# YonghaoHe/LFD-A-Light-and-Fast-Detector

Hardware: AMD Instinct MI355X
Metric: images/sec WIDERFACE-S 1920x1080 bs=8 end-to-end inference, LFD.precision='fp32_storage' (raw logits within 1e-4 of fp32: inside north_star's 1e-3; the 'fp16' mode, sigma 2.5e-3, under fp16_mode) (higher is better)
Workload: dtype f16

## Files before the change

### include/lfd_hip.h

```cpp
#ifndef LFD_HIP_H_
#define LFD_HIP_H_

#include <stddef.h>
#include <stdint.h>

#ifdef __cplusplus
extern "C" {
#endif

#define LFD_HIP_ABI_VERSION 3
#define LFD_MAX_LEVELS 8

typedef void* lfd_stream_t;

#if defined(LFD_BUILDING)
#define LFD_API __attribute__((visibility("default")))
#else
#define LFD_API
#endif

enum lfd_status {
  LFD_OK = 0,
  LFD_ERR_INVALID_ARGUMENT = -1,
  LFD_ERR_WORKSPACE_TOO_SMALL = -2,
// ... 315 lines not shown
  float gn_in_eps;
  int32_t pad_;
  int64_t f_image_stride0, f_image_stride1;
} lfd_pl_head_desc_t;
typedef struct lfd_pl_head_level {
  const void* in;
  void* out;
  const void* w0;
  const float* b0;
  const void* w1;
  const float* b1;
  void* gn_sums;
  const void* gn_in_sums;
  const float* gn_in_gamma;
  const float* gn_in_beta;
  float* f_out0;
  float* f_out1;
  const float* scale1;
  int64_t in_plane_halfs;
  int32_t pixels, pad_;
} lfd_pl_head_level_t;
LFD_API int lfd_pl_head_levels(const lfd_pl_head_desc_t* desc, const lfd_pl_head_level_t* levels, int32_t num_levels,
                               const void* zeros, lfd_stream_t stream);

LFD_API int lfd_stem_conv_f16(const void* in, int32_t in_format, int32_t n, int32_t h, int32_t w,
                              int32_t channels, const void* w1_packed, const float* b1,
                              const void* w2_packed, const float* b2, void* out, lfd_stream_t stream);

LFD_API int lfd_stem_gray_f16(const void* in, int32_t in_format, int32_t n, int32_t h, int32_t w, int32_t channels,
                              const void* w1_packed, const float* b1, const void* w2_packed, const float* b2, void* out,
                              lfd_stream_t stream);
LFD_API int lfd_pl_stem_gray_pair(const void* in, int32_t in_format, int32_t n, int32_t h, int32_t w, int32_t channels,
                                  const void* w1_packed, const float* b1, const void* w2_packed, const float* b2, void* out,
                                  int64_t out_plane_halfs, lfd_stream_t stream);

LFD_API int lfd_stem_faster_fused_f16(const void* in, int32_t in_format, int32_t n, int32_t h, int32_t w,
                                      int32_t channels, const void* w1_packed, const float* b1,
                                      const void* w2_packed, const float* b2, const void* w3_packed,
                                      const float* b3, const void* w4_packed, const float* b4, void* out,
                                      lfd_stream_t stream);

LFD_API size_t lfd_train_workspace_bytes(void);
LFD_API int lfd_pack_conv_weight_train_f16(const float* weight_oihw, int32_t cout, int32_t cin, int32_t ks, int32_t mode,
                                   int32_t rows_valid, void* packed, lfd_stream_t stream);
typedef struct lfd_pack_job {
  const float* w;
// ... 421 lines not shown
```

### lfd-a-light-and-fast-detector_amd/csrc/planes_head.hip

```cpp
#include "planes_impl.h"

namespace pl {

struct PhLevel {
  const void* in;
  long in_plane;
  float* out;
  const half8* w0;
  const float* b0;
  const half8* w1;
  const float* b1;
  unsigned long long* gn_out;
  const unsigned long long* gn_in;
  const float* gamma;
  const float* beta;
  float* f_out0;
  float* f_out1;
  const float* scale1;
  int P, tiles_per_img, tile_start, pad_;
};
struct PhArgs {
  PhLevel lv[LFD_MAX_LEVELS];
  const _Float16* zeros;
  long w_plane0, w_plane1;
  long f_img0, f_img1;
  int n_levels, N, ntiles, relu0;
  int f_c0, f_c1;
  float eps;
};

template <int MODE, int CIN, int NSLAB>
struct PhCfg {
  static constexpr int TPX = 64;
  static constexpr bool PLANES_IN = MODE == 0 || MODE == 3;
  static constexpr int NK0 = (PLANES_IN ? CIN : 128) / 16;
  static constexpr int IN_PIXB = CIN * 2;
  static constexpr int IN_PLANE = TPX * IN_PIXB;
  static constexpr int NBUF = ((MODE == 0 && CIN == 64) || MODE == 3) ? 2 : 1;
  static constexpr int RAW_BYTES = TPX * 512;
  static constexpr int OP_PLANE = TPX * 256;
  static constexpr int IN_OFF = 0;
  static constexpr int IN_BYTES = PLANES_IN ? NBUF * 2 * IN_PLANE : RAW_BYTES;
// ... 416 lines not shown
        const size_t pixi = in_img ? (size_t)px : 0;
        float* q0 = lv.f_out0 + (size_t)n * a.f_img0 + pixi * a.f_c0;
        float* q1 = lv.f_out1 + (size_t)n * a.f_img1 + pixi * a.f_c1 - a.f_c0;
#pragma unroll
        for (int g = 0; g < 4; ++g)
#pragma unroll
          for (int e = 0; e < 4; ++e) {
            if (slab * 32 + 8 * g + e < ctot) {
              const int co = slab * 32 + 8 * g + 4 * h + e;
              const float y = comb(am[0][4 * g + e], ac[0][4 * g + e]);
              const bool first_out = co < a.f_c0;
              float* dst = (in_img && co < ctot) ? (first_out ? q0 : q1) + co : trash;
              *dst = first_out ? y : y * sc1;
            }
          }
      }
    }
    if constexpr (PLANES_IN && C::NBUF == 2) buf ^= 1;
    PH_T(7);
  }
  gn_flush();
}

template <int NSLAB>
__global__ __launch_bounds__(256, 2) void k_pl_head_out(PhArgs a) {
  constexpr int TPX = 64, OP_PLANE = TPX * 256, BIAS_OFF = 4 * OP_PLANE;
  extern __shared__ __attribute__((aligned(16))) char smem[];
  const int lane = threadIdx.x & 63;
  const int wave = __builtin_amdgcn_readfirstlane((int)(threadIdx.x >> 6));
  const int h = lane >> 5, pix = lane & 31;
  const int slab = wave % NSLAB, pt0 = wave / NSLAB;
  const bool mfma_wave = wave < 2 * NSLAB;
  const int pj = (int)threadIdx.x & 31, gi = pj >> 1, prow = (int)threadIdx.x >> 5;
  const int nblk = gridDim.x;
  const int xcd = blockIdx.x & 7, bix = blockIdx.x >> 3;
  const int per_xcd = (a.ntiles + 7) / 8;
  const int x_begin = xcd * per_xcd;
  const int x_end = (x_begin + per_xcd) < a.ntiles ? (x_begin + per_xcd) : a.ntiles;
  const int wgs_xcd = (nblk + 7 - xcd) / 8;
  const int chunk = (x_end - x_begin + wgs_xcd - 1) / (wgs_xcd > 0 ? wgs_xcd : 1);
  const int t_first = x_begin + bix * chunk;
  const int t_last = (t_first + chunk) < x_end ? (t_first + chunk) : x_end;
  int lstart[LFD_MAX_LEVELS];
#pragma unroll
  for (int i = 0; i < LFD_MAX_LEVELS; ++i) lstart[i] = i < a.n_levels ? a.lv[i].tile_start : 0x7fffffff;
  auto level_of = [&](int t) {
    int l = 0;
#pragma unroll
// ... 10 lines not shown
  const char* d_in = nullptr;
  auto load_tile = [&](int t, float4* dst) {
    const int l = level_of(t);
    if (l != d_l) {
      d_l = l;
      with_level(l, [&](const PhLevel& v) { d_in = reinterpret_cast<const char*>(v.in); d_P = v.P; d_tpi = v.tiles_per_img; d_t0 = v.tile_start; });
    }
    const int rel = t - d_t0;
    const int n = rel / d_tpi;
    const int p0 = (rel - n * d_tpi) * TPX;
    const char* base = d_in + (long)n * d_P * 512 + pj * 16;
#pragma unroll
    for (int r = 0; r < 8; ++r) {
      int p = p0 + prow + 8 * r;
      p = p < d_P ? p : d_P - 1;
      dst[r] = *reinterpret_cast<const float4*>(base + (long)p * 512);
    }
  };
  float* sbias = reinterpret_cast<float*>(smem + BIAS_OFF);
  half8 wh[8], wl[8];
  float gn_a[4], gn_b[4];
  PhLevel lv{};
  int cur_l = -1, gnin_key = -1;
  const int xo = (pt0 * 32 + pix) * 256;
  const int xkey = (pix & 15) ^ h;
  float4 cur[8], nxt[8];
  int buf = 0;
  int t = t_first;
  if (t < t_last) load_tile(t, cur);
  for (; t < t_last; ++t, buf ^= 1) {
    const int l = level_of(t);
    if (l != cur_l) {
      cur_l = l;
      with_level(l, [&](const PhLevel& v) { lv = v; });
      const half8* ws = lv.w0 + ((size_t)slab * 8) * 64 + lane;
#pragma unroll
      for (int k = 0; k < 8; ++k) {
        wh[k] = ws[(size_t)k * 64];
        wl[k] = ws[a.w_plane0 + (size_t)k * 64];
      }
      block_barrier();
      if (threadIdx.x < 128) sbias[threadIdx.x] = ((int)threadIdx.x >= NSLAB * 32) ? 0.f : lv.b0[threadIdx.x];
      gnin_key = -1;
    }
    const int rel = t - lv.tile_start;
    const int n = rel / lv.tiles_per_img;
    const int p0 = (rel - n * lv.tiles_per_img) * TPX;
    if (t + 1 < t_last) load_tile(t + 1, nxt);
    if (gnin_key != n) {
      gnin_key = n;
      long long s = 0, q = 0;
#pragma unroll
      for (int r = 0; r < kGnRep; ++r) {
        s += (long long)lv.gn_in[(((size_t)r * a.N + n) * 16 + gi) * 2];
        q += (long long)lv.gn_in[(((size_t)r * a.N + n) * 16 + gi) * 2 + 1];
      }
      const double cnt = (double)lv.P * 8.0;
// ... 33 lines not shown
          ac[4 * g + 0] = 0.f; ac[4 * g + 1] = 0.f; ac[4 * g + 2] = 0.f; ac[4 * g + 3] = 0.f;
        }
      }
      const char* op = smem + buf * 2 * OP_PLANE + xo;
      half8 xh[2], xl[2];
      xh[0] = *reinterpret_cast<const half8*>(op + ((0 ^ xkey) << 4));
      xl[0] = *reinterpret_cast<const half8*>(op + OP_PLANE + ((0 ^ xkey) << 4));
      static_for([&](auto kc) {
        constexpr int k = decltype(kc)::value;
        if constexpr (k + 1 < 8) {
          xh[(k + 1) & 1] = *reinterpret_cast<const half8*>(op + (((2 * (k + 1)) ^ xkey) << 4));
          xl[(k + 1) & 1] = *reinterpret_cast<const half8*>(op + OP_PLANE + (((2 * (k + 1)) ^ xkey) << 4));
        }
        PL_SB();
        am = __builtin_amdgcn_mfma_f32_32x32x16_f16(wh[k], xh[k & 1], am, 0, 0, 0);
        ac = __builtin_amdgcn_mfma_f32_32x32x16_f16(wh[k], xl[k & 1], ac, 0, 0, 0);
        ac = __builtin_amdgcn_mfma_f32_32x32x16_f16(wl[k], xh[k & 1], ac, 0, 0, 0);
        PL_SB();
      }, std::make_integer_sequence<int, 8>{});
      const float sc1 = lv.scale1 ? *lv.scale1 : 1.f;
      const int ctot = a.f_c0 + a.f_c1;
      const int px = p0 + pt0 * 32 + pix;
      const bool in_img = px < lv.P;
      float* q0 = lv.f_out0 + (size_t)n * a.f_img0 + (size_t)px * a.f_c0;
      float* q1 = lv.f_out1 + (size_t)n * a.f_img1 + (size_t)px * a.f_c1 - a.f_c0;
#pragma unroll
      for (int g = 0; g < 4; ++g)
#pragma unroll
        for (int e = 0; e < 4; ++e) {
          if (slab * 32 + 8 * g + e < ctot) {
            const int co = slab * 32 + 8 * g + 4 * h + e;
            const float y = comb(am[4 * g + e], ac[4 * g + e]);
            if (in_img && co < ctot) {
              if (co < a.f_c0) q0[co] = y;
              else q1[co] = y * sc1;
            }
          }
        }
    }
#pragma unroll
    for (int r = 0; r < 8; ++r) cur[r] = nxt[r];
  }
}

template <int NSLAB>
int launch_pl_head_out(PhArgs& a, hipStream_t st) {
  long nt = 0;
  for (int i = 0; i < a.n_levels; ++i) {
    a.lv[i].tiles_per_img = (a.lv[i].P + 63) / 64;
    a.lv[i].tile_start = (int)nt;
    nt += (long)a.N * a.lv[i].tiles_per_img;
    if (nt > 0x7fffffffL) return LFD_ERR_UNSUPPORTED;
  }
  a.ntiles = (int)nt;
  constexpr int LDSB = 4 * 64 * 256 + 512;
  auto kern = k_pl_head_out<NSLAB>;
  static unsigned long long attr_done_mask = 0;
  const int attr_done_dev = lfd_device_ordinal();
  if (LFD_ONCE_PER_DEVICE(attr_done_mask, attr_done_dev)) {
    if (hipFuncSetAttribute(reinterpret_cast<const void*>(kern), hipFuncAttributeMaxDynamicSharedMemorySize, LDSB) != hipSuccess)
      return LFD_ERR_LAUNCH_FAILED;
    LFD_DONE_ON_DEVICE(attr_done_mask, attr_done_dev);
  }
  int blocks = 512;
  if (blocks > 8 * ((a.ntiles + 7) / 8)) blocks = 8 * ((a.ntiles + 7) / 8);
  if (blocks < 1) blocks = 1;
  hipLaunchKernelGGL(kern, dim3(blocks), dim3(256), LDSB, st, a);
  LFD_CHECK_LAUNCH();
  return LFD_OK;
}

__global__ __launch_bounds__(512, 1) void k_pl_head_b2(PhArgs a) {
  constexpr int TPX = 64, OP_PLANE = TPX * 256;
  extern __shared__ __attribute__((aligned(16))) char smem[];
  const int lane = threadIdx.x & 63;
  const int wave = __builtin_amdgcn_readfirstlane((int)(threadIdx.x >> 6));
  const int nblk = gridDim.x;
  const int xcd = blockIdx.x & 7, bix = blockIdx.x >> 3;
  const int per_xcd = (a.ntiles + 7) / 8;
  const int x_begin = xcd * per_xcd;
  const int x_end = (x_begin + per_xcd) < a.ntiles ? (x_begin + per_xcd) : a.ntiles;
  const int wgs_xcd = (nblk + 7 - xcd) / 8;
  const int chunk = (x_end - x_begin + wgs_xcd - 1) / (wgs_xcd > 0 ? wgs_xcd : 1);
  const int t_first = x_begin + bix * chunk;
  const int t_last = (t_first + chunk) < x_end ? (t_first + chunk) : x_end;
  const int nt = t_last > t_first ? t_last - t_first : 0;
  int lstart[LFD_MAX_LEVELS];
#pragma unroll
  for (int i = 0; i < LFD_MAX_LEVELS; ++i) lstart[i] = i < a.n_levels ? a.lv[i].tile_start : 0x7fffffff;
  auto level_of = [&](int t) {
// ... 246 lines not shown
  static unsigned long long attr_done_mask = 0;
  const int attr_done_dev = lfd_device_ordinal();
  if (LFD_ONCE_PER_DEVICE(attr_done_mask, attr_done_dev)) {
    if (hipFuncSetAttribute(reinterpret_cast<const void*>(kern), hipFuncAttributeMaxDynamicSharedMemorySize, C::LDS_BYTES) != hipSuccess)
      return LFD_ERR_LAUNCH_FAILED;
    LFD_DONE_ON_DEVICE(attr_done_mask, attr_done_dev);
  }
  int blocks = 512;
  if (blocks > 8 * ((a.ntiles + 7) / 8)) blocks = 8 * ((a.ntiles + 7) / 8);
  if (blocks < 1) blocks = 1;
  hipLaunchKernelGGL(kern, dim3(blocks), dim3(256), C::LDS_BYTES, st, a);
  LFD_CHECK_LAUNCH();
  return LFD_OK;
}

}

#ifdef LFD_PL_TIMING
extern "C" __attribute__((visibility("default"))) int lfd_debug_pl_head_timing(unsigned long long* host_out) {
  return (int)hipMemcpyFromSymbol(host_out, HIP_SYMBOL(pl::g_pl_dbg), sizeof(unsigned long long) * 136);
}
#endif

extern "C" int lfd_pl_head_levels(const lfd_pl_head_desc_t* d, const lfd_pl_head_level_t* levels, int32_t num_levels, const void* zeros,
                                  lfd_stream_t stream) {
  hipStream_t st = reinterpret_cast<hipStream_t>(stream);
  if (!d || !levels || !zeros || num_levels < 1 || num_levels > LFD_MAX_LEVELS || d->n < 1) return LFD_ERR_INVALID_ARGUMENT;
  if (d->mode < 0 || d->mode > 3) return LFD_ERR_INVALID_ARGUMENT;
  if (d->mode == 0 && d->cin != 64 && d->cin != 128) return LFD_ERR_UNSUPPORTED;
  if (d->mode == 2 && (d->f_c0 < 0 || d->f_c1 < 0 || d->f_c0 + d->f_c1 < 1 || d->f_c0 + d->f_c1 > 64)) return LFD_ERR_UNSUPPORTED;
  pl::PhArgs a{};
  a.zeros = (const _Float16*)zeros;
  a.n_levels = num_levels; a.N = d->n; a.relu0 = d->relu0; a.eps = d->gn_in_eps;
  a.f_c0 = d->f_c0; a.f_c1 = d->f_c1; a.f_img0 = d->f_image_stride0; a.f_img1 = d->f_image_stride1;
  const int nslab0 = d->mode == 2 ? (d->f_c0 + d->f_c1 + 31) / 32 : 4;
  const int nk0 = (d->mode == 0 ? d->cin : 128) / 16;
  a.w_plane0 = (long)nslab0 * nk0 * 64;
  a.w_plane1 = 4L * 8 * 64;
  for (int i = 0; i < num_levels; ++i) {
    const lfd_pl_head_level_t& s = levels[i];
    if (!s.in || !s.w0 || !s.b0 || s.pixels < 1) return LFD_ERR_INVALID_ARGUMENT;
    if (!lfd_aligned16(s.in) || !lfd_aligned16(s.out) || (s.in_plane_halfs & 7)) return LFD_ERR_INVALID_ARGUMENT;
    if (d->mode == 0 && (!s.w1 || !s.b1)) return LFD_ERR_INVALID_ARGUMENT;
    if (d->mode != 2 && (!s.out || !s.gn_sums)) return LFD_ERR_INVALID_ARGUMENT;
    if ((d->mode == 1 || d->mode == 2) && (!s.gn_in_sums || !s.gn_in_gamma || !s.gn_in_beta)) return LFD_ERR_INVALID_ARGUMENT;
    if (d->mode == 2 && ((d->f_c0 > 0 && !s.f_out0) || (d->f_c1 > 0 && !s.f_out1))) return LFD_ERR_INVALID_ARGUMENT;
    pl::PhLevel& l = a.lv[i];
    l.in = s.in; l.in_plane = s.in_plane_halfs; l.out = (float*)s.out;
    l.w0 = (const half8*)s.w0; l.b0 = s.b0; l.w1 = (const half8*)s.w1; l.b1 = s.b1;
    l.gn_out = (unsigned long long*)s.gn_sums; l.gn_in = (const unsigned long long*)s.gn_in_sums;
    l.gamma = s.gn_in_gamma; l.beta = s.gn_in_beta;
    l.f_out0 = s.f_out0; l.f_out1 = s.f_out1; l.scale1 = s.scale1;
    l.P = s.pixels;
  }
  if (d->mode == 0) return d->cin == 64 ? pl::launch_pl_head<0, 64, 4>(a, st) : pl::launch_pl_head<0, 128, 4>(a, st);
  if (d->mode == 3) return pl::launch_pl_head<3, 128, 4>(a, st);
  if (d->mode == 1) return lfd_tune(LFD_TUNE_PL_HEAD_ROLES) != 0 ? pl::launch_pl_head_b2(a, st) : pl::launch_pl_head<1, 128, 4>(a, st);
  if (lfd_tune(LFD_TUNE_PL_HEAD_OUT_REGS) != 0) return nslab0 == 1 ? pl::launch_pl_head_out<1>(a, st) : pl::launch_pl_head_out<2>(a, st);
  return nslab0 == 1 ? pl::launch_pl_head<2, 128, 1>(a, st) : pl::launch_pl_head<2, 128, 2>(a, st);
}
```

### lfd-a-light-and-fast-detector_amd/csrc/postproc.hip

```cpp
#include "common.h"
#include "decode_impl.h"

namespace {

constexpr int kBlock = 256;

struct SegBuffers {
  int cap;
  int words;
  const int* counts;
  int k_host;
  int* total;
  int nclass;
  int* total_ws;
  int class_agnostic;
  float iou_thr;
  float4* cand_box;
  float* cand_score;
  int* cand_label;
  int* cand_point;
  uint32_t* maxord;
  float4* s_box;
  float* s_area;
  float* s_score;
// ... 502 lines not shown
  uint32_t mo = 0u;
  if (i < k) {
    float4 bx = reinterpret_cast<const float4*>(boxes)[i];
    b.cand_box[i] = bx;
    b.cand_score[i] = scores[i];
    b.cand_label[i] = (int)labels[i];
    mo = lfd_float_ord(fmaxf(fmaxf(bx.x, bx.y), fmaxf(bx.z, bx.w)));
  }
#pragma unroll
  for (int s = 32; s > 0; s >>= 1) {
    uint32_t o = __shfl_xor(mo, s, 64);
    mo = o > mo ? o : mo;
  }
  if (lfd_lane() == 0 && mo) atomicMax(&b.maxord[0], mo);
}

__device__ __forceinline__ unsigned long long sort_key(float score, int idx) {
  if (score == 0.f) score = 0.f;
  return ((unsigned long long)(~lfd_float_ord(score)) << 32) | (unsigned)idx;
}

__global__ __launch_bounds__(kBlock) void k_rank_sort(SegBuffers b) {
  __shared__ unsigned long long keys[kBlock];
  const int seg = blockIdx.y;
  const int K = seg_k(b, seg);
  if ((int)(blockIdx.x * kBlock) >= K) return;
  const int64_t so = (int64_t)seg * b.cap;
  const int i = blockIdx.x * kBlock + threadIdx.x;
  const bool live = i < K;
  const float my_score = live ? b.cand_score[so + i] : 0.f;
  auto tie = [&](int j) { return b.total ? b.cand_point[so + j] * b.nclass + b.cand_label[so + j] : j; };
  const unsigned long long my = live ? sort_key(my_score, tie(i)) : ~0ull;
  int rank = 0;
  for (int j0 = 0; j0 < K; j0 += kBlock) {
    const int j = j0 + threadIdx.x;
    __syncthreads();
    keys[threadIdx.x] = j < K ? sort_key(b.cand_score[so + j], tie(j)) : ~0ull;
    __syncthreads();
    const int lim = (K - j0) < kBlock ? (K - j0) : kBlock;
#pragma unroll 8
    for (int t = 0; t < lim; ++t) rank += keys[t] < my;
  }
  if (!live) return;
  const float4 bx = b.cand_box[so + i];
  const int label = b.cand_label[so + i];
  float4 sb = bx;
  if (!b.class_agnostic) {
    const float step = lfd_ord_float(b.maxord[seg]) + 1.0f;
    const float off = (float)label * step;
    sb.x = bx.x + off; sb.y = bx.y + off; sb.z = bx.z + off; sb.w = bx.w + off;
  }
  b.s_idx[so + rank] = i;
  if (b.s_point) b.s_point[so + rank] = b.cand_point[so + i];
  b.s_score[so + rank] = my_score;
  b.s_label[so + rank] = label;
  b.s_box[so + rank] = sb;
  b.s_area[so + rank] = (sb.z - sb.x) * (sb.w - sb.y);
}

__device__ __forceinline__ float bcast(float v, int lane) {
  return __int_as_float(__builtin_amdgcn_readlane(__float_as_int(v), lane));
}

__global__ __launch_bounds__(kBlock) void k_mask(SegBuffers b) {
  __shared__ unsigned short part[4][64];
  const int seg = blockIdx.y;
  const int K = seg_k(b, seg);
  const int nb = (K + 63) >> 6;
  const int64_t so = (int64_t)seg * b.cap;
  const int lane = lfd_lane();
  const int cg = __builtin_amdgcn_readfirstlane((int)(threadIdx.x >> 6));
  const int ntiles = nb * nb;
  const float thr = b.iou_thr;
  for (int t = blockIdx.x; t < ntiles; t += gridDim.x) {
    const int r = t / nb, c = t - r * nb;
// ... 535 lines not shown
```

### lfd-a-light-and-fast-detector_amd/lfd_amd/_lib.py

```python
import ctypes as C
import os

_HERE = os.path.dirname(os.path.abspath(__file__))
LIB_PATH = os.environ.get('LFD_HIP_LIB') or os.path.join(_HERE, 'liblfd_hip.so')
MAX_LEVELS = 8
F32, F16 = 0, 1

_lib = None


class DetectDesc(C.Structure):
    _fields_ = [('num_levels', C.c_int32),
                ('level_h', C.c_int32 * MAX_LEVELS), ('level_w', C.c_int32 * MAX_LEVELS),
                ('level_stride', C.c_int32 * MAX_LEVELS),
                ('level_range_lo', C.c_float * MAX_LEVELS), ('level_range_hi', C.c_float * MAX_LEVELS),
                ('num_classes', C.c_int32), ('num_cls_channels', C.c_int32),
                ('score_mode', C.c_int32), ('decode_mode', C.c_int32),
                ('class_agnostic', C.c_int32), ('max_candidates', C.c_int32),
                ('score_thr', C.c_float), ('iou_thr', C.c_float)]


class DetectExt(C.Structure):
    _fields_ = [('pre_nms_limit', C.c_int32), ('post_nms_limit', C.c_int32)]

# ... 289 lines not shown
    'lfd_stem_faster_fused_f16': (C.c_int, [_P, _I32, _I32, _I32, _I32, _I32, _P, _P, _P, _P, _P, _P, _P, _P, _P, _P]),
    'lfd_head_partial_floats': (_SZ, [C.POINTER(HeadDesc)]),
    'lfd_head_forward_f16': (C.c_int, [C.POINTER(HeadDesc), _I32, C.POINTER(HeadLevelPtrs), _P, _P, _P, _P, _P, _P, _P]),
    'lfd_head_forward_decode_f16': (C.c_int, [C.POINTER(HeadDesc), C.POINTER(HeadLevelPtrs), _P, _P, _P, _P, _P,
                                              C.POINTER(DetectDesc), _P, _P, _SZ, _P]),
    'lfd_groupnorm_finalize': (C.c_int, [C.POINTER(HeadDesc), _P, C.POINTER(C.c_void_p), C.POINTER(C.c_void_p), _F, _P, _P]),
    'lfd_groupnorm_finalize_fold': (C.c_int, [C.POINTER(HeadDesc), _P, C.POINTER(C.c_void_p), C.POINTER(C.c_void_p), _F, _P,
                                              C.POINTER(HeadLevelPtrs), _I32, _P]),
    'lfd_conv_packed_weight_halfs': (_SZ, [_I32, _I32, _I32]),
    'lfd_conv2d_nhwc_f16': (C.c_int, [C.POINTER(ConvDesc), _P, _P, _P, _P, _P, _P, _P, _P, _P]),
    'lfd_fasterblock_fused_f16': (C.c_int, [_I32, _I32, _I32, _P, _P, _P, _P, _P, _P, _P, _P]),
    'lfd_fasterblock128_fused_f16': (C.c_int, [_I32, _I32, _I32, _P, _P, _P, _P, _P, _P, _P]),
    'lfd_downblock_fused_f16': (C.c_int, [_I32, _I32, _I32, _P, _P, _P, _P, _P, _P, _P, _P, _P, _P]),
    'lfd_conv2d_nhwc_f16_acc32': (C.c_int, [C.POINTER(ConvDesc), _P, _P, _P, _P, _P, _P]),
    'lfd_p32_conv_packed_weight_halfs': (_SZ, [_I32, _I32, _I32]),
    'lfd_p32_conv2d_nhwc_f32': (C.c_int, [C.POINTER(P32ConvDesc), _P, _P, _P, _P, _P, _P, _P]),
    'lfd_p32_conv2d_tail_nhwc_f32': (C.c_int, [C.POINTER(P32ConvDesc), _P, _P, _P, _P, _P, _P, _I32, _P]),
    'lfd_pl_stem_pair': (C.c_int, [_P, _I32, _I32, _I32, _I32, _I32, _P, _P, _P, _P, _P, _I64, _P]),
    'lfd_pl_stem2x': (C.c_int, [_P, _I32, _I32, _I32, _I32, _P, _P, _P, _P, _P, _P, _P, _P, _I64, _P, _P]),
    'lfd_pl_conv2d': (C.c_int, [C.POINTER(PlConvDesc), _P, _P, _P, _P, _P, _P, _P, _P, _P, _P, _P, _P, _P, _P, _P, _P, _P, _P, _P]),
    'lfd_pl_block64': (C.c_int, [_I32, _I32, _I32, _P, _I64, _P, _I64, _P, _P, _P, _P, _P, _P]),
    'lfd_pl_conv2d_levels': (C.c_int, [C.POINTER(PlConvDesc), C.POINTER(PlLevel), _I32, _P, _P]),
    'lfd_pl_head_levels': (C.c_int, [C.POINTER(PlHeadDesc), C.POINTER(PlHeadLevel), _I32, _P, _P]),
    'lfd_pl_groupnorm_relu': (C.c_int, [_P, _I64, _I32, _I64, _I32, _P, _P, _P, _F, _I32, _P]),
    'lfd_p32_groupnorm_workspace_bytes': (_SZ, [_I32, _I32]),
    'lfd_p32_groupnorm_relu_f32': (C.c_int, [_P, _I32, _I64, _I32, _I32, _P, _P, _F, _I32, _P, _SZ, _P]),
    'lfd_conv2d_downsample_nhwc_f16': (C.c_int, [C.POINTER(ConvDesc), _P, _P, _P, _P, _P, _P, _P, _P, _P]),
    'lfd_batch_assemble_f32': (C.c_int, [_P, _P, _P, _P, _P, _I32, _I32, _I32, _I32, _I32, _P, _P]),
    'lfd_plan_bbox_crop_batch': (C.c_int, [C.POINTER(PlanDesc), C.POINTER(PlanBufs), _P]),
    'lfd_eval_append_dets_f32': (C.c_int, [C.POINTER(EvalDesc), C.POINTER(EvalBufs), _P, _P, _P, _I32, _I32, _P, _I32, _P, _I32, _P]),
    'lfd_eval_append_rows_f64': (C.c_int, [C.POINTER(EvalDesc), C.POINTER(EvalBufs), _P, _I64, _P, _I32, _P]),
    'lfd_eval_match_workspace_bytes': (_SZ, [C.POINTER(EvalDesc)]),
    'lfd_eval_match': (C.c_int, [C.POINTER(EvalDesc), C.POINTER(EvalBufs), _P, _SZ, _P]),
    'lfd_eval_accumulate_workspace_bytes': (_SZ, [C.POINTER(EvalDesc)]),
    'lfd_eval_accumulate': (C.c_int, [C.POINTER(EvalDesc), C.POINTER(EvalBufs), _P, _SZ, _P]),
    'lfd_eval_tt100k_append_dets_f32': (C.c_int, [C.POINTER(TT100KEvalDesc), C.POINTER(TT100KEvalBufs), _P, _P, _P, _I32, _I32, _P, _I32,
                                                  _P, _P]),
    'lfd_eval_tt100k_append_rows_f64': (C.c_int, [C.POINTER(TT100KEvalDesc), C.POINTER(TT100KEvalBufs), _P, _I64, _P, _I32, _P]),
    'lfd_eval_tt100k_workspace_bytes': (_SZ, [C.POINTER(TT100KEvalDesc)]),
    'lfd_eval_tt100k_match': (C.c_int, [C.POINTER(TT100KEvalDesc), C.POINTER(TT100KEvalBufs), _P, _SZ, _P]),
    'lfd_eval_wf_append_dets_f32': (C.c_int, [C.POINTER(WFEvalDesc), C.POINTER(WFEvalBufs), _P, _P, _P, _I32, _I32, _P, _P]),
    'lfd_eval_wf_append_rows_f64': (C.c_int, [C.POINTER(WFEvalDesc), C.POINTER(WFEvalBufs), _P, _I64, _P]),
    'lfd_eval_wf_workspace_bytes': (_SZ, [C.POINTER(WFEvalDesc)]),
    'lfd_eval_wf_match': (C.c_int, [C.POINTER(WFEvalDesc), C.POINTER(WFEvalBufs), _P, _SZ, _P]),
}

# ... 60 lines not shown
```

### lfd-a-light-and-fast-detector_amd/lfd_amd/engine_p2.py

```python
import ctypes as C
import os

import torch
import torch.nn as nn

from . import _lib, engine, ops
from ._lib import check, lib, ptr, stream_ptr

_UNION = engine._UNION
_LO = 2048.0


class Unsupported(Exception):
    pass


def _split(w):
    w = w.detach().float()
    hi = w.half()
    lo = ((w - hi.float()) * _LO).half()
    return hi, lo


def pack_planes_weight(w):
# ... 30 lines not shown
    out[:, 1, 1, :, 6] = b.detach().float().reshape(c // 32, 32).to(w.device)
    hi, lo = _split(out.reshape(c // 32, 2, 64, 8))
    return torch.stack([hi, lo], 0).contiguous()


def pack_planes_stem2x_tail_weight(w):
    if tuple(w.shape) != (64, 64, 1, 1):
        raise Unsupported('fused stem: first 1x1 must be [64, 64, 1, 1]')
    w2 = w.detach().float().reshape(64, 64)
    idx = torch.empty(4, 2, 8, dtype=torch.long)
    for q in range(4):
        s_, u = q // 2, q % 2
        for hh in range(2):
            for j in range(8):
                idx[q, hh, j] = 32 * s_ + 16 * u + (4 * hh + j if j < 4 else 8 + 4 * hh + j - 4)
    g = w2[:, idx.reshape(-1).to(w2.device)].reshape(2, 32, 4, 2, 8)
    out = g.permute(0, 2, 3, 1, 4).reshape(2, 4, 64, 8)
    hi, lo = _split(out)
    return torch.stack([hi, lo], 0).contiguous()


def _flat_head_enabled():
    return os.environ.get('LFD_P2_FLATHEAD', '1') != '0'


def _stem2x_enabled():
    return os.environ.get('LFD_P2_STEM2X', '1') != '0'


def _block_enabled():
    return os.environ.get('LFD_P2_BLOCK', '1') != '0'


def _pad_bias(b, mult=32):
    n = -(-b.numel() // mult) * mult
    out = b.new_zeros(n, dtype=torch.float32)
    out[:b.numel()] = b.float()
    return out


def to_planes(x):
    hi = x.half()
    return torch.stack([hi, ((x - hi.float()) * _LO).half()], 0).contiguous()


def from_planes(p):
# ... 241 lines not shown
        if len(lens) != 1 or len(self.level_ops) > _lib.MAX_LEVELS:
            return None
        groups = []
        for k in range(lens.pop()):
            by_sig = {}
            for a, _ in self.level_ops:
                o = self.ops[a + k]
                if o.ks != 1 or o.stride != 1 or o.res is not None or o.ds is not None:
                    return None
                sig = (o.cin, o.cout, o.relu, o.tail is not None and o.tail[2], o.out_mode, o.gnin is not None and o.gnin[3],
                       o.f_c0, o.f_c1)
                by_sig.setdefault(sig, []).append(a + k)
            groups.extend(by_sig.values())
        return groups

    def state_for(self, n, h, w, slot=0):
        key = (n, h, w, slot)
        st = self._shape_cache.get(key)
        if st is None:
            st = _State(self, n, h, w)
            self._shape_cache[key] = st
        return st

    def run(self, x, fmt, st):
        if self.num_gn:
            st.gn_sums.zero_()
        fork = _fork_enabled() and len(self.level_ops) > 1 and self.tap_ready[0] + 1 < self.head_start
        if not fork:
            if self.level_groups is not None and _levels_enabled():
                self._launch(x, fmt, st, range(self.head_start))
                self._launch_levels(st)
            else:
                self._launch(x, fmt, st, range(len(self.ops)))
            return
        main = torch.cuda.current_stream()
        a, b = self.level_ops[0]
        self._launch(x, fmt, st, range(0, self.tap_ready[0] + 1))
        st.side.wait_stream(main)
        with torch.cuda.stream(st.side):
            self._launch(x, fmt, st, range(a, b))
        self._launch(x, fmt, st, list(range(self.tap_ready[0] + 1, self.head_start)) + list(range(b, len(self.ops))))
        main.wait_stream(st.side)

    def _desc(self, o, st):
        src = st.bufs[o.src]
        d = _lib.PlConvDesc()
        d.n, d.h, d.w, d.cin, d.cout, d.ks, d.stride, d.relu = st.n, src.shape[2], src.shape[3], o.cin, o.cout, o.ks, o.stride, o.relu
        d.out_mode = o.out_mode
        d.in_plane_halfs = src[0].numel()
        dst = res = dsd = None
        f0 = f1 = None
        if o.out_mode == 2:
            d.f_c0, d.f_c1 = o.f_c0, o.f_c1
            d.f_image_stride0, d.f_image_stride1 = st.P * o.f_c0, st.P * 4
# ... 38 lines not shown
    def _flat_launches(self, modes):
        launches, made_in = [], {}
        for grp, mode in zip(self.level_groups, modes):
            srcs = [self.ops[i].src for i in grp]
            target = None
            if mode in (1, 3):
                for li in range(len(launches) - 1, -1, -1):
                    m2, ops2 = launches[li]
                    if m2 == mode and len(ops2) + len(grp) <= _lib.MAX_LEVELS and all(made_in.get(b_, -1) < li for b_ in srcs):
                        target = li
                        break
                    if any(made_in.get(b_, -1) >= li for b_ in srcs):
                        break
            if target is None:
                launches.append((mode, list(grp)))
                target = len(launches) - 1
            else:
                launches[target][1].extend(grp)
            for i in grp:
                if self.ops[i].dst is not None:
                    made_in[self.ops[i].dst] = target
        return launches

    def _launch_levels_flat(self, st, modes):
        l, sp = lib(), stream_ptr()
        zeros = ptr(ops.zero_line(self.device))
        if st.flat_calls is None:
            calls = []
            for mode, grp in self._flat_launches(modes):
                if mode == 'G':
                    arr = (_lib.PlLevel * len(grp))()
                    d0 = None
                    for j, i in enumerate(grp):
                        o = self.ops[i]
                        d, src, dst, _, _, _, _ = self._desc(o, st)
                        d0 = d0 or d
                        lv = arr[j]
                        lv.in_, lv.out, lv.w_packed, lv.bias = src.data_ptr(), dst.data_ptr(), o.w.data_ptr(), o.b.data_ptr()
                        lv.h, lv.w, lv.in_plane_halfs, lv.out_plane_halfs = src.shape[2], src.shape[3], d.in_plane_halfs, d.out_plane_halfs
                    calls.append(('G', d0, arr, len(grp)))
                    continue
                arr = (_lib.PlHeadLevel * len(grp))()
                d = _lib.PlHeadDesc()
                for j, i in enumerate(grp):
                    o = self.ops[i]
                    src = st.bufs[o.src]
                    lv, gi = arr[j], o.gnin
                    lv.in_, lv.w0, lv.b0 = src.data_ptr(), o.w.data_ptr(), o.b.data_ptr()
                    lv.pixels, lv.in_plane_halfs = src.shape[2] * src.shape[3], src[0].numel()
                    d.mode, d.n, d.cin, d.relu0 = mode, st.n, o.cin, o.relu
                    if mode == 0:
                        lv.w1, lv.b1 = o.tail[0].data_ptr(), o.tail[1].data_ptr()
                    if mode != 2:
                        lv.out, lv.gn_sums = st.bufs[o.dst].data_ptr(), st.gn_sums[o.gn].data_ptr()
                    if gi is not None:
                        lv.gn_in_sums, lv.gn_in_gamma, lv.gn_in_beta = st.gn_sums[gi[0]].data_ptr(), gi[1].data_ptr(), gi[2].data_ptr()
                        d.gn_in_eps = gi[3]
                    if mode == 2:
                        d.f_c0, d.f_c1 = o.f_c0, o.f_c1
                        d.f_image_stride0, d.f_image_stride1 = st.P * o.f_c0, st.P * 4
                        lv.f_out0 = (st.cls.data_ptr() + st.p_off[o.level] * o.f_c0 * 4) if o.f_c0 else None
                        lv.f_out1 = (st.reg.data_ptr() + st.p_off[o.level] * 4 * 4) if o.f_c1 else None
                        lv.scale1 = o.scale.data_ptr() if o.scale is not None else None
                calls.append((mode, d, arr, len(grp)))
            st.flat_calls = calls
        for mode, d, arr, n in st.flat_calls:
            if mode == 'G':
                check(l.lfd_pl_conv2d_levels(C.byref(d), arr, n, zeros, sp), 'lfd_pl_conv2d_levels')
            else:
                check(l.lfd_pl_head_levels(C.byref(d), arr, n, zeros, sp), 'lfd_pl_head_levels')

    def _launch_levels(self, st):
        modes = self._flat_head_modes() if _flat_head_enabled() else None
        if modes is not None:
            return self._launch_levels_flat(st, modes)
        l, sp = lib(), stream_ptr()
        zeros = ptr(ops.zero_line(self.device))
        if st.level_calls is None:
            calls = []
            for grp in self.level_groups:
                arr = (_lib.PlLevel * len(grp))()
                d0 = None
                for j, i in enumerate(grp):
                    o = self.ops[i]
                    d, src, dst, _, _, f0, f1 = self._desc(o, st)
                    d0 = d0 or d
                    lv, gi = arr[j], o.gnin
                    lv.in_, lv.out, lv.w_packed, lv.bias = src.data_ptr(), dst.data_ptr() if dst is not None else None, o.w.data_ptr(), o.b.data_ptr()
                    if o.tail is not None:
                        lv.tail_w_packed, lv.tail_bias = o.tail[0].data_ptr(), o.tail[1].data_ptr()
                    if o.gn is not None:
                        lv.gn_sums = st.gn_sums[o.gn].data_ptr()
                    if gi is not None:
                        lv.gn_in_sums, lv.gn_in_gamma, lv.gn_in_beta = st.gn_sums[gi[0]].data_ptr(), gi[1].data_ptr(), gi[2].data_ptr()
                    lv.f_out0, lv.f_out1 = f0, f1
                    lv.scale1 = o.scale.data_ptr() if o.scale is not None else None
                    lv.h, lv.w, lv.in_plane_halfs, lv.out_plane_halfs = src.shape[2], src.shape[3], d.in_plane_halfs, d.out_plane_halfs
                calls.append((d0, arr, len(grp)))
# ... 97 lines not shown
```

### lfd-a-light-and-fast-detector_amd/lfd_amd/engine_p32.py

```python
import ctypes as C

import torch
import torch.nn as nn

from . import _lib, engine, ops
from ._lib import check, lib, ptr, stream_ptr

_UNION = engine._UNION
_LO = 2048.0


def pack_weight(w):
    w = w.detach().float()
    cout, cin, ks, _ = w.shape
    assert cin % 32 == 0
    ns = -(-cout // 32)
    if ns * 32 != cout:
        w = torch.cat([w, w.new_zeros((ns * 32 - cout, cin, ks, ks))], 0)
    hi = w.half()
    lo = ((w - hi.float()) * _LO).half()

    def frag(t):
        t = t.reshape(ns, 32, cin // 32, 2, 2, 8, ks * ks)
        return t.permute(0, 2, 6, 3, 4, 1, 5)
# ... 246 lines not shown
    if not x.is_contiguous():
        x = x.contiguous()
    fmt, n, h, w = engine._input_format(x, model._backbone._input_channels)
    plan = get_plan(model, x.device)
    st = plan.state_for(n, h, w, slot)
    with torch.cuda.device(x.device):
        if not use_graph:
            plan.run(x, fmt, st)
        else:
            key = (x.data_ptr(), fmt)
            ent = st.graph.get(key)
            if ent is None:
                if len(st.graph) >= 4:
                    st.graph.pop(next(iter(st.graph)))
                plan.run(x, fmt, st)
                torch.cuda.synchronize()
                g = torch.cuda.CUDAGraph()
                with torch.cuda.graph(g):
                    plan.run(x, fmt, st)
                ent = (g, x)
                st.graph[key] = ent
            ent[0].replay()
    return st.cls, st.reg, st.sizes
```

### lfd-a-light-and-fast-detector_amd/lfd_amd/model/lfd.py

```python
import os

import numpy
import torch
import torch.nn as nn
import torch.nn.functional as F

from .. import engine, engine_p32, engine_sibling, ops, parallel, train_engine
from ..data import DeviceAnnotations
from .utils import multiclass_nms

__all__ = ['LFD']

_UNION = ('IoULoss', 'GIoULoss', 'DIoULoss', 'CIoULoss')


class _FusedLossFunction(torch.autograd.Function):

    @staticmethod
    def forward(ctx, pred_cls, pred_reg, cls_t, reg_t, desc, reduce_sums, rank_scale):
        fin = ops.get_loss_forward(desc, pred_cls, pred_reg, cls_t, reg_t, reduce_sums, rank_scale)
        ctx.desc = desc
        ctx.save_for_backward(pred_cls, pred_reg, cls_t, reg_t, fin)
        return fin[:3].clone()

# ... 129 lines not shown
        iou_thr = self._nms_cfg.get('iou_thr', 0.5) if iou_thr is None else iou_thr
        agn = self._nms_cfg.get('class_agnostic', False) if class_agnostic is None else class_agnostic
        cache = self.__dict__.setdefault('_step_graphs', {})
        ver = engine.version_sum(self)
        if self.__dict__.get('_step_graphs_ver') != ver:
            plan = engine_p32.get_plan(self, x.device) if precise else \
                engine.get_plan(self, self._backbone, self._neck, self._head, x.device)
            if self.__dict__.get('_step_graphs_plan') is not plan:
                cache.clear()
                self.__dict__['_step_graphs_plan'] = plan
            self.__dict__['_step_graphs_ver'] = ver
        key = (x.data_ptr(), tuple(x.shape), x.dtype, meta.data_ptr(), float(score_thr), float(iou_thr), bool(agn), max_candidates, slot)
        ent = cache.get(key)
        if ent is None:
            if len(cache) >= 8:
                cache.pop(next(iter(cache)))
            self.use_graph = False
            try:
                with torch.cuda.device(x.device):
                    out = self.detect(self.forward_resident(x, slot), meta, score_thr, iou_thr, agn, max_candidates)
                    torch.cuda.synchronize()
                    desc, _ = self._detect_desc(score_thr, iou_thr, agn, max_candidates)
                    ops.detect_workspace_reset(desc, x.size(0), out)
                    fused = (not precise) and engine.lfd_forward_detect(self, x, desc, meta, out, slot)
                    torch.cuda.synchronize()
                    g = torch.cuda.CUDAGraph()
                    with torch.cuda.graph(g):
                        if fused:
                            engine.lfd_forward_detect(self, x, desc, meta, out, slot)
                        else:
                            cls, reg = self.forward_resident(x, slot)
                            ops.detect_batched(desc, cls, reg, meta, out=out)
            finally:
                self.use_graph = True
            ent = (g, out, x, meta)
            cache[key] = ent
        ent[0].replay()
        return ent[1]

    def _forward_train(self, x):
        neck, head = self._neck, self._head
        hip = x.is_cuda and os.environ.get('LFD_HIP_TRAIN', '1') != '0'
        if hip and train_engine.network_supported(self):
            cls, reg, sizes = train_engine.network_train_forward(self, x)
            for i, sz in enumerate(sizes):
                self._head_indexes_to_feature_map_sizes[i] = sz
            return cls, reg
        if hip and train_engine.supported(self._backbone):
            feats = list(train_engine.backbone_train_forward(self._backbone, x))
        else:
            feats = self._backbone_train_torch(x)
        if type(neck).__name__ == 'SimpleNeck':
# ... 333 lines not shown
```

Measured before the change: 6889.

## Fuse detection decode into flat head output kernel for fp32_storage path

Adds a decoding variant of the flat-tile head output kernel. It thresholds the sigmoid score in-register, decodes candidate boxes and appends them with wave-level atomics straight into the detect workspace, so the fp32 cls/reg maps are never written or re-read by a separate detect pass. The fp32_storage precision path now uses this fused forward+detect when supported. Because candidates arrive in nondeterministic order, rank_sort gains a tie-order computation to restore a deterministic index. The cost is extra atomics and a heavier rank-sort loop.

Measured after the change: 6767. -1.8%, worse.

```diff
diff --git a/include/lfd_hip.h b/include/lfd_hip.h
--- a/include/lfd_hip.h
+++ b/include/lfd_hip.h
@@ -361,6 +361,9 @@
 } lfd_pl_head_level_t;
 LFD_API int lfd_pl_head_levels(const lfd_pl_head_desc_t* desc, const lfd_pl_head_level_t* levels, int32_t num_levels,
                                const void* zeros, lfd_stream_t stream);
+LFD_API int lfd_pl_head_levels_decode(const lfd_pl_head_desc_t* desc, const lfd_pl_head_level_t* levels, int32_t num_levels,
+                                      const void* zeros, const lfd_detect_desc_t* det, const float* img_meta,
+                                      void* det_workspace, size_t det_workspace_bytes, lfd_stream_t stream);
 
 LFD_API int lfd_stem_conv_f16(const void* in, int32_t in_format, int32_t n, int32_t h, int32_t w,
                               int32_t channels, const void* w1_packed, const float* b1,
diff --git a/lfd-a-light-and-fast-detector_amd/csrc/planes_head.hip b/lfd-a-light-and-fast-detector_amd/csrc/planes_head.hip
--- a/lfd-a-light-and-fast-detector_amd/csrc/planes_head.hip
+++ b/lfd-a-light-and-fast-detector_amd/csrc/planes_head.hip
@@ -1,4 +1,6 @@
+#include <type_traits>
 #include "planes_impl.h"
+#include "decode_impl.h"
 
 namespace pl {
 
@@ -17,7 +19,8 @@
   float* f_out0;
   float* f_out1;
   const float* scale1;
-  int P, tiles_per_img, tile_start, pad_;
+  int P, tiles_per_img, tile_start;
+  int p_off;
 };
 struct PhArgs {
   PhLevel lv[LFD_MAX_LEVELS];
@@ -480,8 +483,47 @@
   gn_flush();
 }
 
-template <int NSLAB>
-__global__ __launch_bounds__(256, 2) void k_pl_head_out(PhArgs a) {
+struct PhNoDec {};
+
+__device__ __forceinline__ void ph_decode_append(const LfdAppendTarget& dec, bool pre, float x, float r0, float r1, float r2, float r3hi,
+                                                 int lane, int pix, int n, int q, int point, int lw, int lstride, float lm) {
+#pragma clang fp contract(off)
+  float sc = 0.f;
+  bool cand = false;
+  if (pre) { sc = lfd_sigmoidf_ref(x); cand = sc > dec.score_thr; }
+  const unsigned long long cm = __ballot(cand);
+  if (!cm) return;
+  const float r3 = __shfl(r3hi, pix + 32, 64);
+  const int leader = __ffsll((long long)cm) - 1;
+  int base = 0;
+  if (lane == leader) base = atomicAdd(dec.total + n, (int)__popcll(cm));
+  base = __shfl(base, leader, 64);
+  uint32_t mo = 0u;
+  if (cand) {
+    const int slot = base + (int)__popcll(cm & ((1ull << lane) - 1ull));
+    if (slot < dec.cap) {
+      const int iy = q / lw, ix = q - iy * lw;
+      const float4 box = lfd_decode_core(dec.decode_mode, r0, r1, r2, r3, (float)(ix * lstride), (float)(iy * lstride), lm,
+                                         dec.meta[n * 3 + 0], dec.meta[n * 3 + 1], dec.meta[n * 3 + 2]);
+      const size_t o = (size_t)n * dec.cap + slot;
+      dec.cand_box[o] = box;
+      dec.cand_score[o] = sc;
+      dec.cand_label[o] = 0;
+      dec.cand_point[o] = point;
+      mo = lfd_float_ord(fmaxf(fmaxf(box.x, box.y), fmaxf(box.z, box.w)));
+    }
+  }
+#pragma unroll
+  for (int s = 32; s > 0; s >>= 1) {
+    const uint32_t o = __shfl_xor(mo, s, 64);
+    mo = o > mo ? o : mo;
+  }
+  if (lane == 0 && mo) atomicMax(dec.maxord + n, mo);
+}
+
+template <int NSLAB, bool DEC>
+__global__ __launch_bounds__(256, 2) void k_pl_head_out(PhArgs a, std::conditional_t<DEC, LfdAppendTarget, PhNoDec> dec) {
+  static_assert(!DEC || NSLAB == 1, "the decoding variant: five output channels");
   constexpr int TPX = 64, OP_PLANE = TPX * 256, BIAS_OFF = 4 * OP_PLANE;
   extern __shared__ __attribute__((aligned(16))) char smem[];
   const int lane = threadIdx.x & 63;
@@ -538,6 +580,8 @@
   float gn_a[4], gn_b[4];
   PhLevel lv{};
   int cur_l = -1, gnin_key = -1;
+  int dec_w = 1, dec_stride = 0;
+  float dec_m = 0.f;
   const int xo = (pt0 * 32 + pix) * 256;
   const int xkey = (pix & 15) ^ h;
   float4 cur[8], nxt[8];
@@ -549,6 +593,12 @@
     if (l != cur_l) {
       cur_l = l;
       with_level(l, [&](const PhLevel& v) { lv = v; });
+      if constexpr (DEC) {
+        static_for([&](auto ic) {
+          constexpr int i = decltype(ic)::value;
+          if (l == i) { dec_w = dec.w[i]; dec_stride = dec.stride[i]; dec_m = dec.m[i]; }
+        }, std::make_integer_sequence<int, LFD_MAX_LEVELS>{});
+      }
       const half8* ws = lv.w0 + ((size_t)slab * 8) * 64 + lane;
 #pragma unroll
       for (int k = 0; k < 8; ++k) {
@@ -628,29 +678,37 @@
       const int ctot = a.f_c0 + a.f_c1;
       const int px = p0 + pt0 * 32 + pix;
       const bool in_img = px < lv.P;
-      float* q0 = lv.f_out0 + (size_t)n * a.f_img0 + (size_t)px * a.f_c0;
-      float* q1 = lv.f_out1 + (size_t)n * a.f_img1 + (size_t)px * a.f_c1 - a.f_c0;
-#pragma unroll
-      for (int g = 0; g < 4; ++g)
-#pragma unroll
-        for (int e = 0; e < 4; ++e) {
-          if (slab * 32 + 8 * g + e < ctot) {
-            const int co = slab * 32 + 8 * g + 4 * h + e;
-            const float y = comb(am[4 * g + e], ac[4 * g + e]);
-            if (in_img && co < ctot) {
-              if (co < a.f_c0) q0[co] = y;
-              else q1[co] = y * sc1;
+      if constexpr (DEC) {
+        const float y0 = comb(am[0], ac[0]);
+        const bool pre = h == 0 && in_img && y0 > dec.logit_lo;
+        if (__ballot(pre))
+          ph_decode_append(dec, pre, y0, comb(am[1], ac[1]) * sc1, comb(am[2], ac[2]) * sc1, comb(am[3], ac[3]) * sc1, y0 * sc1,
+                           lane, pix, n, px, lv.p_off + px, dec_w, dec_stride, dec_m);
+      } else {
+        float* q0 = lv.f_out0 + (size_t)n * a.f_img0 + (size_t)px * a.f_c0;
+        float* q1 = lv.f_out1 + (size_t)n * a.f_img1 + (size_t)px * a.f_c1 - a.f_c0;
+#pragma unroll
+        for (int g = 0; g < 4; ++g)
+#pragma unroll
+          for (int e = 0; e < 4; ++e) {
+            if (slab * 32 + 8 * g + e < ctot) {
+              const int co = slab * 32 + 8 * g + 4 * h + e;
+              const float y = comb(am[4 * g + e], ac[4 * g + e]);
+              if (in_img && co < ctot) {
+                if (co < a.f_c0) q0[co] = y;
+                else q1[co] = y * sc1;
+              }
             }
           }
-        }
+      }
     }
 #pragma unroll
     for (int r = 0; r < 8; ++r) cur[r] = nxt[r];
   }
 }
 
-template <int NSLAB>
-int launch_pl_head_out(PhArgs& a, hipStream_t st) {
+template <int NSLAB, bool DEC = false>
+int launch_pl_head_out(PhArgs& a, hipStream_t st, const LfdAppendTarget* dec = nullptr) {
   long nt = 0;
   for (int i = 0; i < a.n_levels; ++i) {
     a.lv[i].tiles_per_img = (a.lv[i].P + 63) / 64;
@@ -660,7 +718,7 @@
   }
   a.ntiles = (int)nt;
   constexpr int LDSB = 4 * 64 * 256 + 512;
-  auto kern = k_pl_head_out<NSLAB>;
+  auto kern = k_pl_head_out<NSLAB, DEC>;
   static unsigned long long attr_done_mask = 0;
   const int attr_done_dev = lfd_device_ordinal();
   if (LFD_ONCE_PER_DEVICE(attr_done_mask, attr_done_dev)) {
@@ -671,7 +729,8 @@
   int blocks = 512;
   if (blocks > 8 * ((a.ntiles + 7) / 8)) blocks = 8 * ((a.ntiles + 7) / 8);
   if (blocks < 1) blocks = 1;
-  hipLaunchKernelGGL(kern, dim3(blocks), dim3(256), LDSB, st, a);
+  if constexpr (DEC) hipLaunchKernelGGL(kern, dim3(blocks), dim3(256), LDSB, st, a, *dec);
+  else hipLaunchKernelGGL(kern, dim3(blocks), dim3(256), LDSB, st, a, PhNoDec{});
   LFD_CHECK_LAUNCH();
   return LFD_OK;
 }
@@ -964,14 +1023,12 @@
 }
 #endif
 
-extern "C" int lfd_pl_head_levels(const lfd_pl_head_desc_t* d, const lfd_pl_head_level_t* levels, int32_t num_levels, const void* zeros,
-                                  lfd_stream_t stream) {
-  hipStream_t st = reinterpret_cast<hipStream_t>(stream);
+static int ph_fill_args(const lfd_pl_head_desc_t* d, const lfd_pl_head_level_t* levels, int32_t num_levels, const void* zeros, bool f_out,
+                        pl::PhArgs& a, int* nslab0_out) {
   if (!d || !levels || !zeros || num_levels < 1 || num_levels > LFD_MAX_LEVELS || d->n < 1) return LFD_ERR_INVALID_ARGUMENT;
   if (d->mode < 0 || d->mode > 3) return LFD_ERR_INVALID_ARGUMENT;
   if (d->mode == 0 && d->cin != 64 && d->cin != 128) return LFD_ERR_UNSUPPORTED;
   if (d->mode == 2 && (d->f_c0 < 0 || d->f_c1 < 0 || d->f_c0 + d->f_c1 < 1 || d->f_c0 + d->f_c1 > 64)) return LFD_ERR_UNSUPPORTED;
-  pl::PhArgs a{};
   a.zeros = (const _Float16*)zeros;
   a.n_levels = num_levels; a.N = d->n; a.relu0 = d->relu0; a.eps = d->gn_in_eps;
   a.f_c0 = d->f_c0; a.f_c1 = d->f_c1; a.f_img0 = d->f_image_stride0; a.f_img1 = d->f_image_stride1;
@@ -979,6 +1036,7 @@
   const int nk0 = (d->mode == 0 ? d->cin : 128) / 16;
   a.w_plane0 = (long)nslab0 * nk0 * 64;
   a.w_plane1 = 4L * 8 * 64;
+  long p_off = 0;
   for (int i = 0; i < num_levels; ++i) {
     const lfd_pl_head_level_t& s = levels[i];
     if (!s.in || !s.w0 || !s.b0 || s.pixels < 1) return LFD_ERR_INVALID_ARGUMENT;
@@ -986,7 +1044,7 @@
     if (d->mode == 0 && (!s.w1 || !s.b1)) return LFD_ERR_INVALID_ARGUMENT;
     if (d->mode != 2 && (!s.out || !s.gn_sums)) return LFD_ERR_INVALID_ARGUMENT;
     if ((d->mode == 1 || d->mode == 2) && (!s.gn_in_sums || !s.gn_in_gamma || !s.gn_in_beta)) return LFD_ERR_INVALID_ARGUMENT;
-    if (d->mode == 2 && ((d->f_c0 > 0 && !s.f_out0) || (d->f_c1 > 0 && !s.f_out1))) return LFD_ERR_INVALID_ARGUMENT;
+    if (d->mode == 2 && f_out && ((d->f_c0 > 0 && !s.f_out0) || (d->f_c1 > 0 && !s.f_out1))) return LFD_ERR_INVALID_ARGUMENT;
     pl::PhLevel& l = a.lv[i];
     l.in = s.in; l.in_plane = s.in_plane_halfs; l.out = (float*)s.out;
     l.w0 = (const half8*)s.w0; l.b0 = s.b0; l.w1 = (const half8*)s.w1; l.b1 = s.b1;
@@ -994,10 +1052,45 @@
     l.gamma = s.gn_in_gamma; l.beta = s.gn_in_beta;
     l.f_out0 = s.f_out0; l.f_out1 = s.f_out1; l.scale1 = s.scale1;
     l.P = s.pixels;
-  }
+    l.p_off = (int)p_off;
+    p_off += s.pixels;
+    if (p_off > 0x7fffffffL) return LFD_ERR_UNSUPPORTED;
+  }
+  *nslab0_out = nslab0;
+  return LFD_OK;
+}
+
+extern "C" int lfd_pl_head_levels(const lfd_pl_head_desc_t* d, const lfd_pl_head_level_t* levels, int32_t num_levels, const void* zeros,
+                                  lfd_stream_t stream) {
+  hipStream_t st = reinterpret_cast<hipStream_t>(stream);
+  pl::PhArgs a{};
+  int nslab0 = 0;
+  const int rc = ph_fill_args(d, levels, num_levels, zeros, true, a, &nslab0);
+  if (rc != LFD_OK) return rc;
   if (d->mode == 0) return d->cin == 64 ? pl::launch_pl_head<0, 64, 4>(a, st) : pl::launch_pl_head<0, 128, 4>(a, st);
   if (d->mode == 3) return pl::launch_pl_head<3, 128, 4>(a, st);
   if (d->mode == 1) return lfd_tune(LFD_TUNE_PL_HEAD_ROLES) != 0 ? pl::launch_pl_head_b2(a, st) : pl::launch_pl_head<1, 128, 4>(a, st);
   if (lfd_tune(LFD_TUNE_PL_HEAD_OUT_REGS) != 0) return nslab0 == 1 ? pl::launch_pl_head_out<1>(a, st) : pl::launch_pl_head_out<2>(a, st);
   return nslab0 == 1 ? pl::launch_pl_head<2, 128, 1>(a, st) : pl::launch_pl_head<2, 128, 2>(a, st);
 }
+
+extern "C" int lfd_pl_head_levels_decode(const lfd_pl_head_desc_t* d, const lfd_pl_head_level_t* levels, int32_t num_levels,
+                                         const void* zeros, const lfd_detect_desc_t* det, const float* img_meta, void* det_workspace,
+                                         size_t det_workspace_bytes, lfd_stream_t stream) {
+  hipStream_t st = reinterpret_cast<hipStream_t>(stream);
+  if (!d || !det || !levels) return LFD_ERR_INVALID_ARGUMENT;
+  if (d->mode != 2 || d->f_c0 != 1 || d->f_c1 != 4) return LFD_ERR_UNSUPPORTED;
+  if (det->num_classes != 1 || det->num_cls_channels != 1 || det->score_mode != 0) return LFD_ERR_UNSUPPORTED;
+  if (det->decode_mode < 0 || det->decode_mode > 3) return LFD_ERR_UNSUPPORTED;
+  if (det->num_levels != num_levels) return LFD_ERR_INVALID_ARGUMENT;
+  pl::PhArgs a{};
+  int nslab0 = 0;
+  int rc = ph_fill_args(d, levels, num_levels, zeros, false, a, &nslab0);
+  if (rc != LFD_OK) return rc;
+  for (int i = 0; i < num_levels; ++i)
+    if ((long)det->level_h[i] * det->level_w[i] != levels[i].pixels) return LFD_ERR_INVALID_ARGUMENT;
+  LfdAppendTarget dec;
+  rc = lfd_detect_bind_append(det, d->n, img_meta, det_workspace, det_workspace_bytes, &dec);
+  if (rc != LFD_OK) return rc;
+  return pl::launch_pl_head_out<1, true>(a, st, &dec);
+}
diff --git a/lfd-a-light-and-fast-detector_amd/csrc/postproc.hip b/lfd-a-light-and-fast-detector_amd/csrc/postproc.hip
--- a/lfd-a-light-and-fast-detector_amd/csrc/postproc.hip
+++ b/lfd-a-light-and-fast-detector_amd/csrc/postproc.hip
@@ -548,6 +548,7 @@
 
 __global__ __launch_bounds__(kBlock) void k_rank_sort(SegBuffers b) {
   __shared__ unsigned long long keys[kBlock];
+  __shared__ unsigned ties[kBlock];
   const int seg = blockIdx.y;
   const int K = seg_k(b, seg);
   if ((int)(blockIdx.x * kBlock) >= K) return;
@@ -556,16 +557,25 @@
   const bool live = i < K;
   const float my_score = live ? b.cand_score[so + i] : 0.f;
   auto tie = [&](int j) { return b.total ? b.cand_point[so + j] * b.nclass + b.cand_label[so + j] : j; };
-  const unsigned long long my = live ? sort_key(my_score, tie(i)) : ~0ull;
-  int rank = 0;
+  const unsigned my_tie = live ? (unsigned)tie(i) : ~0u;
+  const unsigned long long my = live ? sort_key(my_score, (int)my_tie) : ~0ull;
+  const bool appended = b.total != nullptr;
+  int rank = 0, ord = 0;
   for (int j0 = 0; j0 < K; j0 += kBlock) {
     const int j = j0 + threadIdx.x;
     __syncthreads();
-    keys[threadIdx.x] = j < K ? sort_key(b.cand_score[so + j], tie(j)) : ~0ull;
+    const unsigned tj = j < K ? (unsigned)tie(j) : ~0u;
+    keys[threadIdx.x] = j < K ? sort_key(b.cand_score[so + j], (int)tj) : ~0ull;
+    if (appended) ties[threadIdx.x] = tj;
     __syncthreads();
     const int lim = (K - j0) < kBlock ? (K - j0) : kBlock;
+    if (appended) {
 #pragma unroll 8
-    for (int t = 0; t < lim; ++t) rank += keys[t] < my;
+      for (int t = 0; t < lim; ++t) { rank += keys[t] < my; ord += ties[t] < my_tie; }
+    } else {
+#pragma unroll 8
+      for (int t = 0; t < lim; ++t) rank += keys[t] < my;
+    }
   }
   if (!live) return;
   const float4 bx = b.cand_box[so + i];
@@ -576,7 +586,7 @@
     const float off = (float)label * step;
     sb.x = bx.x + off; sb.y = bx.y + off; sb.z = bx.z + off; sb.w = bx.w + off;
   }
-  b.s_idx[so + rank] = i;
+  b.s_idx[so + rank] = appended ? ord : i;
   if (b.s_point) b.s_point[so + rank] = b.cand_point[so + i];
   b.s_score[so + rank] = my_score;
   b.s_label[so + rank] = label;
diff --git a/lfd-a-light-and-fast-detector_amd/lfd_amd/_lib.py b/lfd-a-light-and-fast-detector_amd/lfd_amd/_lib.py
--- a/lfd-a-light-and-fast-detector_amd/lfd_amd/_lib.py
+++ b/lfd-a-light-and-fast-detector_amd/lfd_amd/_lib.py
@@ -335,6 +335,7 @@
     'lfd_pl_block64': (C.c_int, [_I32, _I32, _I32, _P, _I64, _P, _I64, _P, _P, _P, _P, _P, _P]),
     'lfd_pl_conv2d_levels': (C.c_int, [C.POINTER(PlConvDesc), C.POINTER(PlLevel), _I32, _P, _P]),
     'lfd_pl_head_levels': (C.c_int, [C.POINTER(PlHeadDesc), C.POINTER(PlHeadLevel), _I32, _P, _P]),
+    'lfd_pl_head_levels_decode': (C.c_int, [C.POINTER(PlHeadDesc), C.POINTER(PlHeadLevel), _I32, _P, C.POINTER(DetectDesc), _P, _P, _SZ, _P]),
     'lfd_pl_groupnorm_relu': (C.c_int, [_P, _I64, _I32, _I64, _I32, _P, _P, _P, _F, _I32, _P]),
     'lfd_p32_groupnorm_workspace_bytes': (_SZ, [_I32, _I32]),
     'lfd_p32_groupnorm_relu_f32': (C.c_int, [_P, _I32, _I64, _I32, _I32, _P, _P, _F, _I32, _P, _SZ, _P]),
diff --git a/lfd-a-light-and-fast-detector_amd/lfd_amd/engine_p2.py b/lfd-a-light-and-fast-detector_amd/lfd_amd/engine_p2.py
--- a/lfd-a-light-and-fast-detector_amd/lfd_amd/engine_p2.py
+++ b/lfd-a-light-and-fast-detector_amd/lfd_amd/engine_p2.py
@@ -76,6 +76,10 @@
 
 def _flat_head_enabled():
     return os.environ.get('LFD_P2_FLATHEAD', '1') != '0'
+
+
+def _head_decode_enabled():
+    return os.environ.get('LFD_P2_HEAD_DECODE', '1') != '0'
 
 
 def _stem2x_enabled():
@@ -363,14 +367,28 @@
             self._shape_cache[key] = st
         return st
 
-    def run(self, x, fmt, st):
+    def decode_supported(self, st, desc):
+        if not (_head_decode_enabled() and _flat_head_enabled() and _levels_enabled() and self.level_groups is not None):
+            return False
+        if _fork_enabled() and len(self.level_ops) > 1:
+            return False
+        modes = self._flat_head_modes()
+        if modes is None:
+            return False
+        mode, grp = self._flat_launches(modes)[-1]
+        outs = [self.ops[i] for i in grp]
+        return (mode == 2 and [o.level for o in outs] == list(range(len(self.level_ops))) and
+                all(o.f_c0 == 1 and o.f_c1 == 4 for o in outs) and
+                desc.num_classes == 1 and desc.num_cls_channels == 1 and desc.score_mode == 0 and 0 <= desc.decode_mode <= 3)
+
+    def run(self, x, fmt, st, decode=None):
         if self.num_gn:
             st.gn_sums.zero_()
         fork = _fork_enabled() and len(self.level_ops) > 1 and self.tap_ready[0] + 1 < self.head_start
         if not fork:
             if self.level_groups is not None and _levels_enabled():
                 self._launch(x, fmt, st, range(self.head_start))
-                self._launch_levels(st)
+                self._launch_levels(st, decode)
             else:
                 self._launch(x, fmt, st, range(len(self.ops)))
             return
@@ -455,7 +473,7 @@
                     made_in[self.ops[i].dst] = target
         return launches
 
-    def _launch_levels_flat(self, st, modes):
+    def _launch_levels_flat(self, st, modes, decode=None):
         l, sp = lib(), stream_ptr()
         zeros = ptr(ops.zero_line(self.device))
         if st.flat_calls is None:
@@ -497,16 +515,22 @@
                         lv.scale1 = o.scale.data_ptr() if o.scale is not None else None
                 calls.append((mode, d, arr, len(grp)))
             st.flat_calls = calls
-        for mode, d, arr, n in st.flat_calls:
+        for k, (mode, d, arr, n) in enumerate(st.flat_calls):
             if mode == 'G':
                 check(l.lfd_pl_conv2d_levels(C.byref(d), arr, n, zeros, sp), 'lfd_pl_conv2d_levels')
+            elif decode is not None and k == len(st.flat_calls) - 1:
+                ddesc, meta, out = decode
+                check(l.lfd_pl_head_levels_decode(C.byref(d), arr, n, zeros, C.byref(ddesc), ptr(meta), ptr(out.ws), out.ws.numel(), sp),
+                      'lfd_pl_head_levels_decode')
             else:
                 check(l.lfd_pl_head_levels(C.byref(d), arr, n, zeros, sp), 'lfd_pl_head_levels')
 
-    def _launch_levels(self, st):
+    def _launch_levels(self, st, decode=None):
         modes = self._flat_head_modes() if _flat_head_enabled() else None
         if modes is not None:
-            return self._launch_levels_flat(st, modes)
+            return self._launch_levels_flat(st, modes, decode)
+        if decode is not None:
+            raise RuntimeError('the decoding output pass needs the flat-tile head (decode_supported)')
         l, sp = lib(), stream_ptr()
         zeros = ptr(ops.zero_line(self.device))
         if st.level_calls is None:
diff --git a/lfd-a-light-and-fast-detector_amd/lfd_amd/engine_p32.py b/lfd-a-light-and-fast-detector_amd/lfd_amd/engine_p32.py
--- a/lfd-a-light-and-fast-detector_amd/lfd_amd/engine_p32.py
+++ b/lfd-a-light-and-fast-detector_amd/lfd_amd/engine_p32.py
@@ -292,3 +292,19 @@
                 st.graph[key] = ent
             ent[0].replay()
     return st.cls, st.reg, st.sizes
+
+
+def lfd_forward_detect(model, x, desc, meta, out, slot=0):
+    _lib.require_cuda(x, "LFD.forward (precision='fp32_storage')")
+    if not x.is_contiguous():
+        x = x.contiguous()
+    fmt, n, h, w = engine._input_format(x, model._backbone._input_channels)
+    plan = get_plan(model, x.device)
+    decode_supported = getattr(plan, 'decode_supported', None)
+    st = plan.state_for(n, h, w, slot)
+    if decode_supported is None or not decode_supported(st, desc):
+        return False
+    with torch.cuda.device(x.device):
+        plan.run(x, fmt, st, decode=(desc, meta, out))
+        ops.detect_from_candidates(desc, n, out)
+    return True
diff --git a/lfd-a-light-and-fast-detector_amd/lfd_amd/model/lfd.py b/lfd-a-light-and-fast-detector_amd/lfd_amd/model/lfd.py
--- a/lfd-a-light-and-fast-detector_amd/lfd_amd/model/lfd.py
+++ b/lfd-a-light-and-fast-detector_amd/lfd_amd/model/lfd.py
@@ -175,12 +175,13 @@
                     torch.cuda.synchronize()
                     desc, _ = self._detect_desc(score_thr, iou_thr, agn, max_candidates)
                     ops.detect_workspace_reset(desc, x.size(0), out)
-                    fused = (not precise) and engine.lfd_forward_detect(self, x, desc, meta, out, slot)
+                    fwd_detect = engine_p32.lfd_forward_detect if precise else engine.lfd_forward_detect
+                    fused = fwd_detect(self, x, desc, meta, out, slot)
                     torch.cuda.synchronize()
                     g = torch.cuda.CUDAGraph()
                     with torch.cuda.graph(g):
                         if fused:
-                            engine.lfd_forward_detect(self, x, desc, meta, out, slot)
+                            fwd_detect(self, x, desc, meta, out, slot)
                         else:
                             cls, reg = self.forward_resident(x, slot)
                             ops.detect_batched(desc, cls, reg, meta, out=out)
```
